# thangvubk/SoftGroup

Measured on AMD Instinct MI355X. Metric: scans/sec ScanNet-v2-like inference (softgroup_scannet.yaml, full forward_test), higher is better.
Workload: dtype f32

## Files before the change

softgroup_amd/csrc/radix_sort.h:

```cpp
#pragma once
#include <mutex>

#include "common.h"
#include "scan.h"

namespace sg {

constexpr int kRsBlock = 256;
constexpr int kRsItems = 8;
constexpr int kRsTile = kRsBlock * kRsItems;
constexpr int kRsBuckets = 256;

inline size_t radix_sort_workspace_bytes(int64_t n) {
  const int64_t nblk = (n + kRsTile - 1) / kRsTile;
  const int64_t hist = nblk * kRsBuckets + 1;
  return align_up(hist * 4) + align_up(scan_workspace_bytes(hist) + 4 * kRsBuckets * 4) +
         2 * align_up(n * 4) + 256;
}

static __global__ void __launch_bounds__(kRsBlock) rs_hist_kernel(const uint32_t *__restrict__ keys,
                                                          int64_t n, int shift, int nblk, int items,
                                                          int32_t *__restrict__ hist,
                                                          int32_t *totals) {
  __shared__ int h[kRsBuckets];
// ... 99 lines not shown
  }
  __syncthreads();
  for (int e = threadIdx.x; e < in_tile; e += kRsBlock) {
    const uint32_t key = skey[e];
    const int d = (key >> shift) & 0xff;
    const int off = base[d] + (e - dstart[d]);
    keys_out[off] = key;
    vals_out[off] = sval[e];
  }
}


static inline int radix_sort_pairs(uint32_t *keys, int32_t *vals, int64_t n, int num_bits, void *ws,
                            size_t ws_bytes, hipStream_t stream, uint32_t **keys_sorted,
                            int32_t **vals_sorted) {
  *keys_sorted = keys;
  *vals_sorted = vals;
  if (n <= 1 || num_bits <= 0) return SG_OK;
  if (ws_bytes < radix_sort_workspace_bytes(n)) {
    set_error("radix_sort_pairs: workspace too small");
    return SG_ERR_WORKSPACE;
  }
  int items = kRsItems;
  while (items < 64 && (n + static_cast<int64_t>(items) * kRsBlock - 1) / (static_cast<int64_t>(items) * kRsBlock) > 256)
    items *= 2;
  const int64_t tile = static_cast<int64_t>(items) * kRsBlock;
  const int nblk = static_cast<int>((n + tile - 1) / tile);
  const size_t lds = static_cast<size_t>(tile) * 8;
  {
    static std::mutex mu;
    static uint64_t done_mask = 0;
    int dev = 0;
    hipGetDevice(&dev);
    std::lock_guard<std::mutex> g(mu);
    if (dev < 0 || dev >= 64 || !((done_mask >> dev) & 1)) {
      if (hipFuncSetAttribute(reinterpret_cast<const void *>(rs_scatter_kernel),
                              hipFuncAttributeMaxDynamicSharedMemorySize, 64 * kRsBlock * 8) != hipSuccess) {
        (void)hipGetLastError();
        set_error("radix_sort_pairs: %d bytes of dynamic LDS are not available on this device (gfx950: 160 KB "
                  "per workgroup)", 64 * kRsBlock * 8);
        return SG_ERR_LAUNCH;
      }
      if (dev >= 0 && dev < 64) done_mask |= 1ull << dev;
    }
  }
  const int64_t hist_n = static_cast<int64_t>(nblk) * kRsBuckets;
  Workspace a(ws, ws_bytes);
  int32_t *hist = a.take<int32_t>(hist_n + 1);
  const size_t sbytes = scan_workspace_bytes(hist_n) + 4 * kRsBuckets * 4;
  void *sws = a.take<char>(sbytes);
  uint32_t *k2 = a.take<uint32_t>(n);
  int32_t *v2 = a.take<int32_t>(n);
  uint32_t *kin = keys, *kout = k2;
  int32_t *vin = vals, *vout = v2;
  const int n_pass = (num_bits + 7) / 8;
  const bool local_scan = nblk <= 256 && n_pass <= 4;
  int32_t *totals = static_cast<int32_t *>(sws);
  if (local_scan) hipMemsetAsync(totals, 0, static_cast<size_t>(n_pass) * kRsBuckets * 4, stream);
  for (int shift = 0, pass = 0; shift < num_bits; shift += 8, ++pass) {
    if (local_scan) {
      int32_t *t = totals + pass * kRsBuckets;
      rs_hist_kernel<<<nblk, kRsBlock, 0, stream>>>(kin, n, shift, nblk, items, hist, t);
      rs_scatter_kernel<<<nblk, kRsBlock, lds, stream>>>(kin, vin, n, shift, nblk, items, hist, t, kout, vout);
      if (const int rc = check_launch("radix_sort_pairs(scatter)"); rc != SG_OK) return rc;
    } else {
      rs_hist_kernel<<<nblk, kRsBlock, 0, stream>>>(kin, n, shift, nblk, items, hist, nullptr);
      int32_t *h = hist;
      int rc = exclusive_scan([h] __device__(int64_t i) { return h[i]; },
                              [h] __device__(int64_t i, int v) { h[i] = v; }, hist_n, nullptr, sws,
                              sbytes, stream);
      if (rc != SG_OK) return rc;
      rs_scatter_kernel<<<nblk, kRsBlock, lds, stream>>>(kin, vin, n, shift, nblk, items, hist, nullptr,
                                                         kout, vout);
      if (const int rc = check_launch("radix_sort_pairs(scatter)"); rc != SG_OK) return rc;
    }
    uint32_t *tk = kin; kin = kout; kout = tk;
    int32_t *tv = vin; vin = vout; vout = tv;
  }
  *keys_sorted = kin;
  *vals_sorted = vin;
  return check_launch("radix_sort_pairs");
}

}
```

softgroup_amd/csrc/spconv_rulebook.hip:

```cpp
#include <stdlib.h>

#include <mutex>

#include "common.h"
#include "radix_sort.h"
#include "scan.h"

namespace sg {

constexpr uint64_t kKeyEmpty = ~0ULL;

struct HashWs {
  uint64_t *keys;
  int32_t *vals;
  int32_t *owner, *rank;
  void *scan_ws;
  size_t scan_bytes;
  uint32_t cap;
};

static size_t hash_cap(int n) {
  size_t cap = 1024;
  while (cap < static_cast<size_t>(n) * 2) cap <<= 1;
  return cap;
// ... 186 lines not shown
    const int sl = slot[t];
    if (sl < 0 || vals[static_cast<size_t>(l) * cap + sl] != i) continue;
    const int r = pos[t] - pos[static_cast<size_t>(l) * M0];
    rowtab[static_cast<size_t>(l) * cap + sl] = r;
    const int4 c = reinterpret_cast<const int4 *>(indices0)[i];
    if (o.indices[l] != nullptr)
      reinterpret_cast<int4 *>(o.indices[l])[r] = make_int4(c.x, c.y >> l, c.z >> l, c.w >> l);
  }
}

__global__ void __launch_bounds__(256) pyr_link_kernel(const int32_t *__restrict__ indices0, int M0,
                                                      int L, const int32_t *__restrict__ vals,
                                                      const int32_t *__restrict__ rowtab,
                                                      uint32_t cap, const int32_t *__restrict__ slot,
                                                      const int32_t *__restrict__ pos, PyrOut o) {
  const int64_t total = static_cast<int64_t>(L - 1) * M0;
  for (int64_t t = blockIdx.x * 256LL + threadIdx.x; t < total; t += gridDim.x * 256LL) {
    const int l = static_cast<int>(t / M0), i = static_cast<int>(t - static_cast<int64_t>(l) * M0);
    const int sl = slot[t];
    if (sl < 0 || vals[static_cast<size_t>(l) * cap + sl] != i) continue;
    const int j = pos[t] - pos[static_cast<size_t>(l) * M0];
    const int s2 = slot[t + M0];
    const int up = s2 >= 0 ? rowtab[static_cast<size_t>(l + 1) * cap + s2] : -1;
    const int4 c = reinterpret_cast<const int4 *>(indices0)[i];
    const int k = (((c.y >> l) & 1) << 2) | (((c.z >> l) & 1) << 1) | ((c.w >> l) & 1);
    o.in2out[l][j] = up;
    if (up >= 0) o.child[l][static_cast<int64_t>(up) * 8 + k] = j;
    int4 *dst = reinterpret_cast<int4 *>(o.inv[l] + static_cast<int64_t>(j) * 8);
    dst[0] = make_int4(k == 0 ? up : -1, k == 1 ? up : -1, k == 2 ? up : -1, k == 3 ? up : -1);
    dst[1] = make_int4(k == 4 ? up : -1, k == 5 ? up : -1, k == 6 ? up : -1, k == 7 ? up : -1);
  }
}

__global__ void __launch_bounds__(256) pyr_subm_kernel(int L, const uint64_t *__restrict__ keys,
                                                      const int32_t *__restrict__ rowtab,
                                                      uint32_t cap, PyrOut o) {
  const long long total = o.pre27[L];
  int l = 0;
  for (long long t = blockIdx.x * 256LL + threadIdx.x; t < total; t += gridDim.x * 256LL) {
    while (t >= o.pre27[l + 1]) ++l;
    const long long e = t - o.pre27[l];
    const int j = static_cast<int>(e / 27), k = static_cast<int>(e - static_cast<long long>(j) * 27);
    const int4 c = reinterpret_cast<const int4 *>(o.indices[l])[j];
    const Shape3 s = o.shape[l];
    const int x = c.y + k / 9 - 1, y = c.z + (k / 3) % 3 - 1, z = c.w + k % 3 - 1;
    int32_t r = -1;
    if (k == 13) r = j;
    else if (x >= 0 && y >= 0 && z >= 0 && x < s.s0 && y < s.s1 && z < s.s2)
      r = hash_find(keys + static_cast<size_t>(l) * cap, rowtab + static_cast<size_t>(l) * cap, cap - 1,
                    lin_key(c.x, x, y, z, s));
    o.nbr[l][e] = r;
  }
}

struct PlanSeg {
  const int32_t *nbr;
  int32_t *order;
  uint32_t *tile_mask;
  int32_t *nbr_tiles;
  int rows, K, row_base, tile_base, sb_base, sb_rows;
  int key_bits, seg_code;
  const uint32_t *key_sorted;
  const int32_t *val_sorted;
};
struct PlanSegs {
  int n, total_rows, total_tiles, total_sbs;
  int n_big, big_rows;
  int n_wide, wide_rows;
  PlanSeg s[kPyrMaxSegs];
};

constexpr int kSbRowsMax = 16384;
constexpr int kSbIndexBits = 14;
static int plan_sb_rows(int rows) {
  static const int env = getenv("SG_PLAN_SB") ? atoi(getenv("SG_PLAN_SB")) : 0;
  int sb = env > 0 ? env : (rows + 7) / 8;
  if (env <= 0 && sb < 4096) sb = 4096;
  sb = (sb + 31) / 32 * 32;
  if (sb < 32) sb = 32;
  if (sb > kSbRowsMax) sb = kSbRowsMax;
  return sb;
}

__global__ void __launch_bounds__(1024) plan_sort_sb_kernel(PlanSegs P, const uint32_t *__restrict__ mask,
                                                           const int32_t *__restrict__ bitpos,
                                                           int32_t *__restrict__ val_sorted,
                                                           uint32_t *__restrict__ tmask) {
  extern __shared__ __attribute__((aligned(16))) uint64_t e[];
  __shared__ int pos[32];
  int seg = P.n_big;
  while (seg + 1 < P.n && static_cast<int>(blockIdx.x) >= P.s[seg + 1].sb_base) ++seg;
  const PlanSeg &S = P.s[seg];
  const int sb = blockIdx.x - S.sb_base;
  const int first = sb * S.sb_rows;
  const int cnt = min(S.sb_rows, S.rows - first);
  const int K = S.K;
  if (threadIdx.x < 32) pos[threadIdx.x] = bitpos[seg * 32 + threadIdx.x];
  int N = 64;
  while (N < cnt) N <<= 1;
  __syncthreads();
  for (int i = threadIdx.x; i < N; i += 1024) {
    uint64_t v = ~0ull;
    if (i < cnt) {
      uint32_t key = 0;
      for (uint32_t mm = mask[S.row_base + first + i]; mm; mm &= mm - 1) key |= 1u << pos[__ffs(static_cast<int>(mm)) - 1];
      v = (static_cast<uint64_t>(key) << kSbIndexBits) | static_cast<uint64_t>(i);
    }
    e[i] = v;
  }
  __syncthreads();
  for (int k = 2; k <= N; k <<= 1) {
    for (int j = k >> 1; j > 0; j >>= 1) {
      for (int t = threadIdx.x; t < N / 2; t += 1024) {
        const int i = 2 * t - (t & (j - 1));
        const int l = i + j;
        const uint64_t a = e[i], b = e[l];
        const bool up = (i & k) == 0;
        if ((a > b) == up) { e[i] = b; e[l] = a; }
      }
      __syncthreads();
    }
  }
  for (int i0 = 0; i0 < N; i0 += 1024) {
    const int i = i0 + threadIdx.x;
    uint32_t key = 0;
    if (i < cnt) {
      const uint64_t v = e[i];
      val_sorted[S.row_base + first + i] = first + static_cast<int>(v & ((1u << kSbIndexBits) - 1u));
      key = static_cast<uint32_t>(v >> kSbIndexBits);
    }
#pragma unroll
    for (int o = 16; o > 0; o >>= 1) key |= __shfl_xor(key, o, 64);
    if ((threadIdx.x & 31) == 0 && i < cnt) {
      uint32_t m = 0;
      for (int k = 0; k < K; ++k) m |= ((key >> pos[k]) & 1u) << k;
      tmask[S.tile_base + sb * (S.sb_rows >> 5) + (i >> 5)] = m;
    }
  }
}

__global__ void __launch_bounds__(1024) plan_tile_order_xcd_kernel(PlanSegs P, const uint32_t *__restrict__ tmask,
                                                                  int mode, int32_t *__restrict__ torder) {
  __shared__ int bucket[4096];
  __shared__ int hist[33];
  const PlanSeg &S = P.s[blockIdx.x];
  const int nt = (S.rows + 31) / 32;
  const int x = blockIdx.y, q = nt >> 3, r = nt & 7;
  const int cnt = q + (x < r ? 1 : 0), start = x * q + min(x, r);
  if (x == 0) {
    if (threadIdx.x < 33) hist[threadIdx.x] = 0;
    __syncthreads();
    for (int t = threadIdx.x; t < nt; t += 1024) atomicAdd(&hist[__popc(tmask[S.tile_base + t])], 1);
    __syncthreads();
    if (threadIdx.x < SG_PLAN_HIST_WORDS) S.tile_mask[nt + threadIdx.x] = threadIdx.x < 33 ? hist[threadIdx.x] : 0;
  }
  const int sb_tiles = S.sb_rows >> 5;
  const int sb0 = start / sb_tiles;
  auto bucket_of = [&](int t) {
    const int b = 32 - __popc(tmask[S.tile_base + t]);
    return mode == 2 ? (t / sb_tiles - sb0) * 33 + b : b;
  };
  for (int c0 = 0; c0 < cnt; c0 += 4096) {
    const int n = min(4096, cnt - c0);
    __syncthreads();
    for (int i = threadIdx.x; i < n; i += 1024) bucket[i] = bucket_of(start + c0 + i);
    __syncthreads();
    for (int i = threadIdx.x; i < n; i += 1024) {
      const int bi = bucket[i];
      int rank = 0;
      for (int j = 0; j < n; ++j) {
        const int bj = bucket[j];
        rank += (bj < bi || (bj == bi && j < i)) ? 1 : 0;
      }
      torder[S.tile_base + (c0 + rank) * 8 + x] = start + c0 + i;
    }
  }
}

__global__ void __launch_bounds__(256) plan_mask_all_kernel(PlanSegs P, uint32_t *__restrict__ mask,
                                                           int32_t *__restrict__ val,
                                                           int32_t *__restrict__ freq) {
  __shared__ int cnt[32];
  const int seg = blockIdx.y;
  const int rows = P.s[seg].rows, K = P.s[seg].K, row_base = P.s[seg].row_base;
  if (blockIdx.x * 256 >= rows) return;
  const int32_t *nbr = P.s[seg].nbr;
  if (threadIdx.x < 32) cnt[threadIdx.x] = 0;
  __syncthreads();
  const int j = blockIdx.x * 256 + threadIdx.x;
  uint32_t m = 0;
  if (j < rows) {
    const int32_t *row = nbr + static_cast<int64_t>(j) * K;
    for (int k = 0; k < K; ++k) m |= (row[k] >= 0 ? 1u : 0u) << k;
    mask[row_base + j] = m;
    val[row_base + j] = row_base + j;
  }
  for (int k = 0; k < K; ++k) {
    const int c = __popcll(__ballot((m >> k) & 1u));
    if ((threadIdx.x & 63) == 0 && c) atomicAdd(&cnt[k], c);
  }
  __syncthreads();
  if (threadIdx.x < K && cnt[threadIdx.x]) atomicAdd(&freq[seg * 32 + threadIdx.x], cnt[threadIdx.x]);
}

__global__ void plan_pos_all_kernel(PlanSegs P, const int32_t *__restrict__ freq, int32_t *__restrict__ bitpos) {
  const int seg = blockIdx.x, k = threadIdx.x;
  const int K = P.s[seg].K;
  int p = 0;
  if (k < K) {
    const int fk = freq[seg * 32 + k];
    for (int o = 0; o < K; ++o) {
      const int fo = freq[seg * 32 + o];
      p += (fo > fk || (fo == fk && o < k)) ? 1 : 0;
    }
  }
  bitpos[seg * 32 + k] = p;
}

__global__ void __launch_bounds__(256) plan_key_all_kernel(PlanSegs P, const int32_t *__restrict__ bitpos,
                                                          uint32_t *__restrict__ mask_to_key) {
  __shared__ int pos[32];
  const int seg = blockIdx.y;
  const int rows = P.s[seg].rows;
  if (blockIdx.x * 256 >= rows) return;
  if (threadIdx.x < 32) pos[threadIdx.x] = bitpos[seg * 32 + threadIdx.x];
  __syncthreads();
  const int j = blockIdx.x * 256 + threadIdx.x;
  if (j >= rows) return;
  const int g = P.s[seg].row_base + j;
  uint32_t key = 0;
  for (uint32_t mm = mask_to_key[g]; mm; mm &= mm - 1) key |= 1u << pos[__ffs(static_cast<int>(mm)) - 1];
  mask_to_key[g] = key | (static_cast<uint32_t>(P.s[seg].seg_code) << P.s[seg].key_bits);
}

__global__ void __launch_bounds__(256) plan_tiles_all_kernel(PlanSegs P, const int32_t *__restrict__ bitpos,
                                                            uint32_t *__restrict__ tmask) {
  __shared__ int pos[32];
  const int seg = blockIdx.y;
  const int rows = P.s[seg].rows, K = P.s[seg].K;
  if (blockIdx.x * 256 >= rows) return;
  if (threadIdx.x < 32) pos[threadIdx.x] = bitpos[seg * 32 + threadIdx.x];
  __syncthreads();
  const int j = blockIdx.x * 256 + threadIdx.x;
  uint32_t key = j < rows ? P.s[seg].key_sorted[P.s[seg].row_base + j] & ((1u << P.s[seg].key_bits) - 1u) : 0u;
#pragma unroll
  for (int o = 16; o > 0; o >>= 1) key |= __shfl_xor(key, o, 64);
  if ((threadIdx.x & 31) == 0 && j < rows) {
    uint32_t m = 0;
    for (int k = 0; k < K; ++k) m |= ((key >> pos[k]) & 1u) << k;
    tmask[P.s[seg].tile_base + (j >> 5)] = m;
  }
}

__global__ void __launch_bounds__(1024) plan_tile_order_all_kernel(PlanSegs P, const uint32_t *__restrict__ tmask,
                                                                  int32_t *__restrict__ torder) {
  __shared__ int hist[33], base[33];
  __shared__ int wcnt[16][33];
  const PlanSeg &S = P.s[blockIdx.x];
  const int nt = (S.rows + 31) / 32;
  const int wave = threadIdx.x >> 6, lane = threadIdx.x & 63;
  if (threadIdx.x < 33) hist[threadIdx.x] = 0;
  __syncthreads();
  for (int t = threadIdx.x; t < nt; t += 1024) atomicAdd(&hist[__popc(tmask[S.tile_base + t])], 1);
  __syncthreads();
  if (threadIdx.x == 0) {
    int run = 0;
    for (int b = 32; b >= 0; --b) { base[b] = run; run += hist[b]; }
  }
  if (threadIdx.x < SG_PLAN_HIST_WORDS) S.tile_mask[nt + threadIdx.x] = threadIdx.x < 33 ? hist[threadIdx.x] : 0;
  __syncthreads();
  for (int t0 = 0; t0 < nt; t0 += 1024) {
    if (threadIdx.x < 16 * 33) (&wcnt[0][0])[threadIdx.x] = 0;
    __syncthreads();
    const int t = t0 + threadIdx.x;
    const bool valid = t < nt;
    const int b = valid ? __popc(tmask[S.tile_base + t]) : 0;
    uint64_t peers = __ballot(valid);
#pragma unroll
    for (int bit = 0; bit < 6; ++bit) {
      const uint64_t bal = __ballot((b >> bit) & 1);
      peers &= ((b >> bit) & 1) ? bal : ~bal;
    }
    const int lane_rank = __popcll(peers & ((1ull << lane) - 1ull));
    if (valid && lane_rank == 0) wcnt[wave][b] = __popcll(peers);
    __syncthreads();
    if (valid) {
      int off = base[b] + lane_rank;
      for (int w = 0; w < wave; ++w) off += wcnt[w][b];
      torder[S.tile_base + off] = t;
    }
    __syncthreads();
    if (threadIdx.x < 33) {
      int add = 0;
      for (int w = 0; w < 16; ++w) add += wcnt[w][threadIdx.x];
      base[threadIdx.x] += add;
    }
    __syncthreads();
  }
}

__global__ void __launch_bounds__(256) plan_emit_all_kernel(PlanSegs P, const int32_t *__restrict__ val_local,
                                                           const uint32_t *__restrict__ tmask,
                                                           const int32_t *__restrict__ torder) {
  const int seg = blockIdx.y;
  const int rows = P.s[seg].rows, K = P.s[seg].K, tile_base = P.s[seg].tile_base;
  const int val_base = P.s[seg].row_base;
  const bool local_vals = seg >= P.n_big;
  const int32_t *val_sorted = local_vals ? val_local : P.s[seg].val_sorted;
  const int row_base = local_vals ? 0 : val_base;
  const int nt = (rows + 31) / 32, per_tile = 32 * K;
  const int32_t *nbr = P.s[seg].nbr;
  int32_t *order = P.s[seg].order, *nbr_tiles = P.s[seg].nbr_tiles;
  uint32_t *tile_mask = P.s[seg].tile_mask;
  for (int t2 = blockIdx.x; t2 < nt; t2 += gridDim.x) {
    const int t = torder[tile_base + t2];
    if (threadIdx.x == 0) tile_mask[t2] = tmask[tile_base + t];
    if (threadIdx.x < 32) {
      const int pos = t * 32 + threadIdx.x;
      order[t2 * 32 + threadIdx.x] = pos < rows ? val_sorted[val_base + pos] - row_base : -1;
    }
    for (int e = threadIdx.x; e < per_tile; e += 256) {
      const int r = e / K, k = e - r * K;
      const int pos = t * 32 + r;
      nbr_tiles[static_cast<int64_t>(t2) * per_tile + e] =
          pos < rows ? nbr[static_cast<int64_t>(val_sorted[val_base + pos] - row_base) * K + k] : -1;
    }
  }
}

static size_t plan_scratch_bytes(size_t R, size_t T) {
  return 2 * align_up(R * 4) + 2 * align_up(T * 4) + 2 * align_up(kPyrMaxSegs * 32 * 4) +
         radix_sort_workspace_bytes(static_cast<int64_t>(R)) + 512;
}

static int plan_order_mode() {
  static const int mode = getenv("SG_PLAN_ORDER") ? atoi(getenv("SG_PLAN_ORDER")) : 0;
  return mode;
}
static void finalize_segs(PlanSegs &P) {
  const int mode = plan_order_mode();
  PlanSeg big[kPyrMaxSegs], small[kPyrMaxSegs];
  int nb = 0, ns = 0;
  P.n_wide = 0;
  P.wide_rows = 0;
  if (mode == 0) {
    for (int i = 0; i < P.n; ++i)
      if (P.s[i].K > 8) big[nb++] = P.s[i];
    P.n_wide = nb;
    for (int i = 0; i < P.n; ++i)
      if (P.s[i].K <= 8) big[nb++] = P.s[i];
    for (int i = 0; i < nb; ++i) {
      big[i].key_bits = i < P.n_wide ? static_cast<int>(kPlanKeyBits) : 8;
      big[i].seg_code = i < P.n_wide ? i : i - P.n_wide;
    }
  } else {
    for (int i = 0; i < P.n; ++i) small[ns++] = P.s[i];
  }
  int row_base = 0, tile_base = 0, sb_base = 0;
  P.n_big = nb;
  for (int i = 0; i < P.n; ++i) {
    PlanSeg &S = P.s[i];
    S = i < nb ? big[i] : small[i - nb];
    S.row_base = row_base;
    S.tile_base = tile_base;
    S.sb_base = sb_base;
    S.sb_rows = mode == 0 ? (S.rows + 31) / 32 * 32 : plan_sb_rows(S.rows);
    row_base += S.rows;
    tile_base += (S.rows + 31) / 32;
    if (i >= nb) sb_base += (S.rows + S.sb_rows - 1) / S.sb_rows;
    if (i + 1 == nb) P.big_rows = row_base;
    if (i + 1 == P.n_wide) P.wide_rows = row_base;
  }
  if (nb == 0) P.big_rows = 0;
  P.total_rows = row_base;
  P.total_tiles = tile_base;
  P.total_sbs = sb_base;
}

static int build_plans(const PlanSegs &P, void *ws2, size_t ws2_bytes, bool zero_freq, hipStream_t stream,
                       const char *who) {
  Workspace wsp(ws2, ws2_bytes);
  const size_t R = static_cast<size_t>(P.total_rows);
  uint32_t *mask = wsp.take<uint32_t>(R);
  int32_t *val = wsp.take<int32_t>(R);
  uint32_t *tmask = wsp.take<uint32_t>(P.total_tiles);
  int32_t *torder = wsp.take<int32_t>(P.total_tiles);
  int32_t *freq = wsp.take<int32_t>(kPyrMaxSegs * 32);
  int32_t *bitpos = wsp.take<int32_t>(kPyrMaxSegs * 32);
  const size_t rs_bytes = radix_sort_workspace_bytes(static_cast<int64_t>(R));
  void *rs_ws = wsp.take<char>(rs_bytes);
  if (!rs_ws) {
    set_error("%s: build workspace too small", who);
    return SG_ERR_WORKSPACE;
  }
  if (zero_freq) hipMemsetAsync(freq, 0, kPyrMaxSegs * 32 * 4, stream);
  int max_rows = 0, max_big = 0;
  for (int i = 0; i < P.n; ++i) {
    max_rows = P.s[i].rows > max_rows ? P.s[i].rows : max_rows;
    if (i < P.n_big) max_big = P.s[i].rows > max_big ? P.s[i].rows : max_big;
  }
  const dim3 grid((max_rows + 255) / 256, P.n);
  plan_mask_all_kernel<<<grid, 256, 0, stream>>>(P, mask, val, freq);
  static const bool raw_env = getenv("SG_PLAN_RAW") != nullptr;
  if (raw_env) hipMemsetAsync(freq, 0, kPyrMaxSegs * 32 * 4, stream);
  plan_pos_all_kernel<<<P.n, 32, 0, stream>>>(P, freq, bitpos);
  const int mode = plan_order_mode();
  PlanSegs Q = P;
  if (P.n_big > 0) {
    const dim3 gbig((max_big + 255) / 256, P.n_big);
    plan_key_all_kernel<<<gbig, 256, 0, stream>>>(P, bitpos, mask);
    struct Group { int first, count, row0, rows, key_bits; } groups[2] = {
        {0, P.n_wide, 0, P.wide_rows, static_cast<int>(kPlanKeyBits)},
        {P.n_wide, P.n_big - P.n_wide, P.wide_rows, P.big_rows - P.wide_rows, 8}};
    for (const Group &g : groups) {
      if (g.count == 0 || g.rows == 0) continue;
      int nbits = g.key_bits;
      for (int n = g.count - 1; n > 0; n >>= 1) ++nbits;
      uint32_t *ms;
      int32_t *vs;
      int rc = radix_sort_pairs(mask + g.row0, val + g.row0, static_cast<int64_t>(g.rows), nbits, rs_ws, rs_bytes,
                                stream, &ms, &vs);
      if (rc != SG_OK) return rc;
      if (ms != mask + g.row0) {
        hipMemcpyAsync(mask + g.row0, ms, static_cast<size_t>(g.rows) * 4, hipMemcpyDeviceToDevice, stream);
        hipMemcpyAsync(val + g.row0, vs, static_cast<size_t>(g.rows) * 4, hipMemcpyDeviceToDevice, stream);
      }
      for (int i = g.first; i < g.first + g.count; ++i) {
        Q.s[i].key_sorted = mask;
        Q.s[i].val_sorted = val;
      }
    }
    plan_tiles_all_kernel<<<gbig, 256, 0, stream>>>(Q, bitpos, tmask);
  }
  if (P.total_sbs > 0) {
    int max_sb = 64;
    for (int i = P.n_big; i < P.n; ++i)
      while (max_sb < P.s[i].sb_rows && max_sb < P.s[i].rows) max_sb <<= 1;
    static std::once_flag once;
    std::call_once(once, [] {
      hipFuncSetAttribute(reinterpret_cast<const void *>(plan_sort_sb_kernel), hipFuncAttributeMaxDynamicSharedMemorySize,
                          kSbRowsMax * 8);
    });
    plan_sort_sb_kernel<<<P.total_sbs, 1024, static_cast<size_t>(max_sb) * 8, stream>>>(Q, mask, bitpos, val, tmask);
  }
  if (mode == 0) plan_tile_order_all_kernel<<<P.n, 1024, 0, stream>>>(Q, tmask, torder);
  else plan_tile_order_xcd_kernel<<<dim3(P.n, 8), 1024, 0, stream>>>(Q, tmask, mode, torder);
  plan_emit_all_kernel<<<dim3(min((max_rows + 31) / 32, 2048), P.n), 256, 0, stream>>>(Q, val, tmask, torder);
  return check_launch(who);
}

struct PyrWs {
  uint64_t *keys;
  int32_t *vals;
  int32_t *rowtab;
  int32_t *slot;
  int32_t *pos;
  void *scan_ws;
  size_t scan_bytes;
  uint32_t cap;
};
static bool pyr_carve(void *ws, size_t ws_bytes, int M0, int L, PyrWs *w) {
  Workspace a(ws, ws_bytes);
  const size_t nn = static_cast<size_t>(M0 > 0 ? M0 : 1);
  w->cap = static_cast<uint32_t>(hash_cap(M0));
  w->keys = a.take<uint64_t>(static_cast<size_t>(L) * w->cap);
  w->vals = a.take<int32_t>(static_cast<size_t>(L) * w->cap);
  w->rowtab = a.take<int32_t>(static_cast<size_t>(L) * w->cap);
  w->slot = a.take<int32_t>(static_cast<size_t>(L) * nn);
  w->pos = a.take<int32_t>(static_cast<size_t>(L) * nn + 1);
  w->scan_bytes = scan_workspace_bytes(static_cast<int64_t>(L) * nn);
  w->scan_ws = a.take<char>(w->scan_bytes);
  return w->scan_ws != nullptr;
}

}

using namespace sg;

extern "C" {

size_t sg_spconv_hash_workspace_bytes(int M) {
  const size_t nn = static_cast<size_t>(M > 0 ? M : 1);
  return align_up(hash_cap(M) * 8) + align_up(hash_cap(M) * 4) + 3 * align_up(nn * 4) +
         align_up(scan_workspace_bytes(M)) + 256;
}

static int build_hash_common(HashWs *w, void *ws, size_t ws_bytes, int M, hipStream_t stream,
                             const char *who) {
  if (!hash_carve(ws, ws_bytes, M, w)) {
    set_error("%s: workspace too small", who);
    return SG_ERR_WORKSPACE;
  }
  hipMemsetAsync(w->keys, 0xff, static_cast<size_t>(w->cap) * 8, stream);
  hipMemsetAsync(w->vals, 0x7f, static_cast<size_t>(w->cap) * 4, stream);
  return SG_OK;
}

int sg_spconv_subm_rulebook(const int32_t *indices, int M, const int32_t *shape_host, int32_t *nbr,
                            void *ws, size_t ws_bytes, sg_stream_t stream_) {
  SG_REQUIRE(M >= 0 && shape_host, "sg_spconv_subm_rulebook: bad arguments");
  if (M == 0) return SG_OK;
  hipStream_t stream = as_stream(stream_);
  HashWs w;
  int rc = build_hash_common(&w, ws, ws_bytes, M, stream, "sg_spconv_subm_rulebook");
  if (rc != SG_OK) return rc;
  const Shape3 shape{shape_host[0], shape_host[1], shape_host[2]};
  subm_insert_kernel<<<(M + 255) / 256, 256, 0, stream>>>(indices, M, shape, w.keys, w.vals,
                                                         w.cap - 1);
  subm_lookup_kernel<<<grid_for(static_cast<int64_t>(M) * 27, 256, 256 * 32), 256, 0, stream>>>(
      indices, M, shape, w.keys, w.vals, w.cap - 1, nbr);
  return check_launch("sg_spconv_subm_rulebook");
}

int sg_spconv_down_build(const int32_t *indices, int M, const int32_t *shape_host, int32_t *in2out,
                         int32_t *meta, void *ws, size_t ws_bytes, sg_stream_t stream_) {
  SG_REQUIRE(M >= 0 && shape_host, "sg_spconv_down_build: bad arguments");
  hipStream_t stream = as_stream(stream_);
  hipMemsetAsync(meta, 0, 4, stream);
  if (M == 0) return SG_OK;
  HashWs w;
  int rc = build_hash_common(&w, ws, ws_bytes, M, stream, "sg_spconv_down_build");
  if (rc != SG_OK) return rc;
  const Shape3 oshape{shape_host[0] / 2, shape_host[1] / 2, shape_host[2] / 2};
  const int grid = (M + 255) / 256;
  int32_t *slot_of = w.rank;
  down_insert_kernel<<<grid, 256, 0, stream>>>(indices, M, oshape, w.keys, w.vals, w.cap - 1,
// ... 73 lines not shown
  const int m0 = M0;
  const uint32_t cap = w.cap;
  const int64_t n = static_cast<int64_t>(L) * M0;
  int rc = exclusive_scan(
      [slot, vals, m0, cap] __device__(int64_t t) {
        const int64_t l = t / m0;
        const int sl = slot[t];
        return (sl >= 0 && vals[l * cap + sl] == static_cast<int32_t>(t - l * m0)) ? 1 : 0;
      },
      [pos] __device__(int64_t t, int v) { pos[t] = v; }, n, pos + n, w.scan_ws, w.scan_bytes, stream);
  if (rc != SG_OK) return rc;
  pyr_rows_kernel<<<1, 64, 0, stream>>>(w.pos, M0, L, rows_dev);
  return check_launch("sg_spconv_pyramid_rows");
}

static long long pyr_seg_rows(const sg_pyramid_level *lv, int L, int seg_kind, int l) {
  return seg_kind == 1 ? lv[l + 1].rows : lv[l].rows;
}

size_t sg_spconv_pyramid_build_workspace_bytes(const sg_pyramid_level *levels, int n_levels) {
  long long total = 0;
  for (int l = 0; l < n_levels; ++l) {
    total += levels[l].rows;
    if (l + 1 < n_levels) total += levels[l + 1].rows + levels[l].rows;
  }
  const size_t R = static_cast<size_t>(total > 0 ? total : 1);
  const size_t T = R / 32 + static_cast<size_t>(3 * n_levels) + 1;
  return plan_scratch_bytes(R, T);
}

int sg_spconv_pyramid_build(const int32_t *indices, int M0, const int32_t *shape_host, int n_levels,
                            const sg_pyramid_level *levels, void *ws, size_t ws_bytes, void *ws2,
                            size_t ws2_bytes, sg_stream_t stream_) {
  SG_REQUIRE(M0 >= 0 && shape_host && levels && n_levels >= 1 && n_levels <= kPyrMaxLevels,
             "sg_spconv_pyramid_build: bad arguments (M0=%d n_levels=%d)", M0, n_levels);
  SG_REQUIRE(levels[0].rows == M0, "sg_spconv_pyramid_build: levels[0].rows must be num_rows");
  if (M0 == 0) return SG_OK;
  hipStream_t stream = as_stream(stream_);
  const int L = n_levels;
  PyrWs w;
  if (!pyr_carve(ws, ws_bytes, M0, L, &w)) {
    set_error("sg_spconv_pyramid_build: workspace too small (%zu bytes)", ws_bytes);
    return SG_ERR_WORKSPACE;
  }
  SG_REQUIRE(ws2 != nullptr && ws2_bytes >= sg_spconv_pyramid_build_workspace_bytes(levels, L),
             "sg_spconv_pyramid_build: build workspace too small (%zu bytes)", ws2_bytes);
  PyrOut o;
  PlanSegs P;
  P.n = 0;
  auto add_seg = [&](const int32_t *nbr, int rows, int K, const sg_plan_ptrs &pl) {
    PlanSeg &S = P.s[P.n++];
    S.nbr = nbr; S.order = pl.order; S.tile_mask = pl.tile_mask; S.nbr_tiles = pl.nbr_tiles;
    S.rows = rows; S.K = K;
  };
  Shape3 s{shape_host[0], shape_host[1], shape_host[2]};
  o.pre27[0] = 0;
  for (int l = 0; l < kPyrMaxLevels; ++l) {
    const bool in = l < L;
    o.indices[l] = in ? levels[l].indices : nullptr;
    o.nbr[l] = in ? levels[l].nbr : nullptr;
    o.in2out[l] = in ? levels[l].in2out : nullptr;
    o.child[l] = in ? levels[l].child : nullptr;
    o.inv[l] = in ? levels[l].inv : nullptr;
    o.shape[l] = s;
    o.pre27[l + 1] = o.pre27[l] + (in ? static_cast<long long>(levels[l].rows) * 27 : 0);
    s = Shape3{s.s0 / 2, s.s1 / 2, s.s2 / 2};
  }
  for (int l = 0; l < L; ++l) {
    SG_REQUIRE(levels[l].rows >= 0 && levels[l].nbr && levels[l].indices && levels[l].subm.order,
               "sg_spconv_pyramid_build: level %d: missing output pointers", l);
    if (l + 1 < L)
      SG_REQUIRE(levels[l].in2out && levels[l].child && levels[l].inv && levels[l].down.order &&
                     levels[l].up.order, "sg_spconv_pyramid_build: level %d: missing output pointers", l);
  }
  for (int l = 0; l < L; ++l) {
    if (levels[l].rows > 0) add_seg(levels[l].nbr, levels[l].rows, 27, levels[l].subm);
    if (l + 1 < L) {
      if (levels[l + 1].rows > 0) add_seg(levels[l].child, levels[l + 1].rows, 8, levels[l].down);
      if (levels[l].rows > 0) add_seg(levels[l].inv, levels[l].rows, 8, levels[l].up);
    }
  }
  if (P.n == 0) return check_launch("sg_spconv_pyramid_build");
  finalize_segs(P);
  int32_t *freq;
  {
    Workspace wsp(ws2, ws2_bytes);
    const size_t R = static_cast<size_t>(P.total_rows);
    wsp.take<uint32_t>(R);
    wsp.take<int32_t>(R);
    wsp.take<uint32_t>(P.total_tiles);
    wsp.take<int32_t>(P.total_tiles);
    freq = wsp.take<int32_t>(kPyrMaxSegs * 32);
    if (!freq) {
      set_error("sg_spconv_pyramid_build: build workspace too small");
      return SG_ERR_WORKSPACE;
    }
  }
  {
    static_assert(kPyrMaxLevels + 1 <= kFillMax, "one fill region per level + the histogram");
    FillList f;
    for (int l = 0; l + 1 < L; ++l)
      if (levels[l + 1].rows > 0) f.add(levels[l].child, static_cast<size_t>(levels[l + 1].rows) * 8 * 4, 0xff);
    f.add(freq, kPyrMaxSegs * 32 * 4, 0);
    fill_many(f, stream);
  }
  const int g_all = grid_for(static_cast<int64_t>(L) * M0, 256, 4096);
  pyr_emit_kernel<<<g_all, 256, 0, stream>>>(indices, M0, L, w.vals, w.rowtab, w.cap, w.slot, w.pos, o);
  if (L > 1) {
    pyr_link_kernel<<<grid_for(static_cast<int64_t>(L - 1) * M0, 256, 4096), 256, 0, stream>>>(
        indices, M0, L, w.vals, w.rowtab, w.cap, w.slot, w.pos, o);
  }
  pyr_subm_kernel<<<grid_for(o.pre27[L], 256, 8192), 256, 0, stream>>>(L, w.keys, w.rowtab, w.cap, o);
  return build_plans(P, ws2, ws2_bytes, false, stream, "sg_spconv_pyramid_build");
}

size_t sg_spconv_plan_workspace_bytes(int M) {
  const size_t nn = static_cast<size_t>(M > 0 ? M : 1);
  return plan_scratch_bytes(nn, (nn + 31) / 32 + 1);
}

int sg_spconv_plan(const int32_t *nbr, int M, int K, int32_t *order, uint32_t *tile_mask,
                   int32_t *nbr_tiles, void *ws, size_t ws_bytes, sg_stream_t stream_) {
  SG_REQUIRE(M >= 0 && K >= 1 && K <= 27, "sg_spconv_plan: bad arguments (M=%d K=%d)", M, K);
  if (M == 0) return SG_OK;
  PlanSegs P;
  P.n = 1;
  P.s[0] = PlanSeg{nbr, order, tile_mask, nbr_tiles, M, K, 0, 0, 0, 0, 0, 0, nullptr, nullptr};
  finalize_segs(P);
  return build_plans(P, ws, ws_bytes, true, as_stream(stream_), "sg_spconv_plan");
}

}
```

Measured before the change: 435.7.

## Use segmented radix sort for plan keys and fold bit-position kernel into consumers

Adds a segmented radix sort that sorts each plan segment's keys inside its own row range. This drops the segment-code high bits from the key, so fewer radix passes are needed and each pass uses 512 or 256 buckets. Per-segment totals are zeroed up front, in the existing fill for the pyramid build or in a memset otherwise. The separate plan_pos_all kernel is removed, and each consuming kernel now recomputes the frequency-ranked bit positions locally. The cost is a linear search over segments in every workgroup and redundant per-block rank computation.

Measured after the change: 437.0 (median of 3 runs). Within noise of the previous version (+0.3%).

```diff
diff --git a/softgroup_amd/csrc/radix_sort.h b/softgroup_amd/csrc/radix_sort.h
--- a/softgroup_amd/csrc/radix_sort.h
+++ b/softgroup_amd/csrc/radix_sort.h
@@ -205,4 +205,230 @@
   return check_launch("radix_sort_pairs");
 }
 
-}
+constexpr int kRsSegMax = 32;
+constexpr int kRsSegMaxWgs = 256;
+struct RsSegs {
+  int n, items;
+  int row0[kRsSegMax + 1];
+  int wg0[kRsSegMax + 1];
+};
+inline bool rs_segs_layout(const int *rows, int n, RsSegs *S) {
+  if (n < 1 || n > kRsSegMax) return false;
+  for (int items = kRsItems; items <= 64; items *= 2) {
+    const int64_t tile = static_cast<int64_t>(items) * kRsBlock;
+    int64_t wgs = 0, row = 0;
+    for (int s = 0; s < n; ++s) {
+      S->row0[s] = static_cast<int>(row);
+      S->wg0[s] = static_cast<int>(wgs);
+      row += rows[s];
+      wgs += (rows[s] + tile - 1) / tile;
+    }
+    if (row >= (1ll << 31)) return false;
+    S->row0[n] = static_cast<int>(row);
+    S->wg0[n] = static_cast<int>(wgs);
+    S->n = n;
+    S->items = items;
+    if (wgs <= kRsSegMaxWgs) return true;
+  }
+  return false;
+}
+inline size_t rs_seg_hist_words(int bits) { return static_cast<size_t>(kRsSegMaxWgs) << bits; }
+inline size_t rs_seg_total_words(int n_seg, int num_bits, int bits) {
+  return static_cast<size_t>((num_bits + bits - 1) / bits) * n_seg * (static_cast<size_t>(1) << bits);
+}
+
+template <int BITS>
+static __global__ void __launch_bounds__(kRsBlock) rs_seg_hist_kernel(const uint32_t *__restrict__ keys, RsSegs S,
+                                                                      int shift, int32_t *__restrict__ hist,
+                                                                      int32_t *totals) {
+  constexpr int NB = 1 << BITS, PER = NB / kRsBlock;
+  __shared__ int h[NB];
+#pragma unroll
+  for (int q = 0; q < PER; ++q) h[threadIdx.x + q * kRsBlock] = 0;
+  __syncthreads();
+  const int wg = blockIdx.x;
+  int s = 0;
+  while (s + 1 < S.n && wg >= S.wg0[s + 1]) ++s;
+  const int wl = wg - S.wg0[s], nblk = S.wg0[s + 1] - S.wg0[s];
+  const int tile = S.items * kRsBlock;
+  const int first = S.row0[s] + wl * tile;
+  const int end = min(first + tile, S.row0[s + 1]);
+  for (int i = first + threadIdx.x; i < end; i += kRsBlock) atomicAdd(&h[(keys[i] >> shift) & (NB - 1)], 1);
+  __syncthreads();
+#pragma unroll
+  for (int q = 0; q < PER; ++q) {
+    const int d = threadIdx.x + q * kRsBlock;
+    const int c = h[d];
+    hist[static_cast<int64_t>(NB) * S.wg0[s] + static_cast<int64_t>(d) * nblk + wl] = c;
+    if (c) atomicAdd(&totals[s * NB + d], c);
+  }
+}
+
+template <int BITS>
+static __global__ void __launch_bounds__(kRsBlock) rs_seg_scatter_kernel(const uint32_t *__restrict__ keys,
+                                                                         const int32_t *__restrict__ vals, RsSegs S,
+                                                                         int shift, const int32_t *__restrict__ hist,
+                                                                         const int32_t *__restrict__ totals,
+                                                                         uint32_t *__restrict__ keys_out,
+                                                                         int32_t *__restrict__ vals_out) {
+  constexpr int NB = 1 << BITS, PER = NB / kRsBlock;
+  extern __shared__ __attribute__((aligned(16))) unsigned char rs_lds[];
+  const int items = S.items;
+  uint32_t *skey = reinterpret_cast<uint32_t *>(rs_lds);
+  int32_t *sval = reinterpret_cast<int32_t *>(rs_lds) + items * kRsBlock;
+  __shared__ int base[NB];
+  __shared__ int dstart[NB];
+  __shared__ int run[NB];
+  __shared__ int wcnt[4][NB];
+  __shared__ int lds4[4];
+  const int wave = threadIdx.x >> 6, lane = threadIdx.x & 63;
+  const int wg = blockIdx.x;
+  int s = 0;
+  while (s + 1 < S.n && wg >= S.wg0[s + 1]) ++s;
+  const int wl = wg - S.wg0[s], nblk = S.wg0[s + 1] - S.wg0[s];
+  const int tile = S.row0[s] + wl * items * kRsBlock;
+  const int in_tile = min(items * kRsBlock, S.row0[s + 1] - tile);
+#pragma unroll
+  for (int q = 0; q < PER; ++q) run[threadIdx.x + q * kRsBlock] = 0;
+  __syncthreads();
+  for (int e = threadIdx.x; e < in_tile; e += kRsBlock) atomicAdd(&run[(keys[tile + e] >> shift) & (NB - 1)], 1);
+  __syncthreads();
+  {
+    int mine[PER], sum = 0;
+#pragma unroll
+    for (int q = 0; q < PER; ++q) { mine[q] = run[threadIdx.x * PER + q]; sum += mine[q]; }
+    int excl = block_incl_scan_256(sum, lds4, nullptr) - sum;
+#pragma unroll
+    for (int q = 0; q < PER; ++q) { dstart[threadIdx.x * PER + q] = excl; excl += mine[q]; }
+  }
+  {
+    int tot[PER], before[PER], sum = 0;
+#pragma unroll
+    for (int q = 0; q < PER; ++q) {
+      const int d = threadIdx.x * PER + q;
+      const int32_t *row = hist + static_cast<int64_t>(NB) * S.wg0[s] + static_cast<int64_t>(d) * nblk;
+      int bf = 0, b = 0;
+      for (; b + 16 <= wl; b += 16) {
+        int v[16];
+#pragma unroll
+        for (int u = 0; u < 16; ++u) v[u] = row[b + u];
+#pragma unroll
+        for (int u = 0; u < 16; ++u) bf += v[u];
+      }
+      for (; b < wl; ++b) bf += row[b];
+      before[q] = bf;
+      tot[q] = totals[s * NB + d];
+      sum += tot[q];
+    }
+    int excl = block_incl_scan_256(sum, lds4, nullptr) - sum;
+#pragma unroll
+    for (int q = 0; q < PER; ++q) { base[threadIdx.x * PER + q] = S.row0[s] + excl + before[q]; excl += tot[q]; }
+  }
+#pragma unroll
+  for (int q = 0; q < PER; ++q) run[threadIdx.x + q * kRsBlock] = 0;
+  __syncthreads();
+  uint32_t pk[8];
+  int32_t pv[8];
+  for (int r = 0; r < items; ++r) {
+    if ((r & 7) == 0) {
+#pragma unroll
+      for (int q = 0; q < 8; ++q) {
+        const int e = (r + q) * kRsBlock + threadIdx.x;
+        pk[q] = e < in_tile ? keys[tile + e] : 0u;
+        pv[q] = e < in_tile ? vals[tile + e] : 0;
+      }
+    }
+#pragma unroll
+    for (int w = 0; w < 4; ++w)
+#pragma unroll
+      for (int q = 0; q < PER; ++q) wcnt[w][threadIdx.x + q * kRsBlock] = 0;
+    __syncthreads();
+    const bool valid = r * kRsBlock + static_cast<int>(threadIdx.x) < in_tile;
+    uint32_t key = 0u;
+    int32_t val = 0;
+#pragma unroll
+    for (int q = 0; q < 8; ++q)
+      if ((r & 7) == q) { key = pk[q]; val = pv[q]; }
+    const int d = (key >> shift) & (NB - 1);
+    uint64_t peers = __ballot(valid);
+#pragma unroll
+    for (int b = 0; b < BITS; ++b) {
+      const uint64_t bal = __ballot((d >> b) & 1);
+      peers &= ((d >> b) & 1) ? bal : ~bal;
+    }
+    const int lane_rank = __popcll(peers & ((1ull << lane) - 1ull));
+    if (valid && lane_rank == 0) wcnt[wave][d] = __popcll(peers);
+    __syncthreads();
+    if (valid) {
+      int off = dstart[d] + run[d] + lane_rank;
+      for (int w = 0; w < wave; ++w) off += wcnt[w][d];
+      skey[off] = key;
+      sval[off] = val;
+    }
+    __syncthreads();
+#pragma unroll
+    for (int q = 0; q < PER; ++q) {
+      const int dd = threadIdx.x + q * kRsBlock;
+      run[dd] += wcnt[0][dd] + wcnt[1][dd] + wcnt[2][dd] + wcnt[3][dd];
+    }
+  }
+  __syncthreads();
+  const int seg_lo = S.row0[s], seg_hi = S.row0[s + 1];
+  for (int e = threadIdx.x; e < in_tile; e += kRsBlock) {
+    const uint32_t key = skey[e];
+    const int d = (key >> shift) & (NB - 1);
+    const int off = base[d] + (e - dstart[d]);
+    if (off >= seg_lo && off < seg_hi) {
+      keys_out[off] = key;
+      vals_out[off] = sval[e];
+    }
+  }
+}
+
+template <int BITS>
+static inline int radix_sort_pairs_segmented(uint32_t *keys, int32_t *vals, uint32_t *keys2, int32_t *vals2,
+                                             const RsSegs &S, int num_bits, int32_t *hist, int32_t *totals,
+                                             hipStream_t stream, uint32_t **keys_sorted, int32_t **vals_sorted) {
+  static_assert(BITS == 8 || BITS == 9, "256 or 512 buckets at 256 threads");
+  constexpr int NB = 1 << BITS;
+  *keys_sorted = keys;
+  *vals_sorted = vals;
+  if (S.row0[S.n] <= 0 || num_bits <= 0) return SG_OK;
+  const int nwg = S.wg0[S.n];
+  if (nwg < 1 || nwg > kRsSegMaxWgs || S.items > 64) {
+    set_error("radix_sort_pairs_segmented: %d workgroups of %d rounds", nwg, S.items);
+    return SG_ERR_ARG;
+  }
+  const size_t lds = static_cast<size_t>(S.items) * kRsBlock * 8;
+  {
+    static std::mutex mu;
+    static uint64_t done_mask = 0;
+    int dev = 0;
+    hipGetDevice(&dev);
+    std::lock_guard<std::mutex> g(mu);
+    if (dev < 0 || dev >= 64 || !((done_mask >> dev) & 1)) {
+      if (hipFuncSetAttribute(reinterpret_cast<const void *>(rs_seg_scatter_kernel<BITS>),
+                              hipFuncAttributeMaxDynamicSharedMemorySize, 64 * kRsBlock * 8) != hipSuccess) {
+        (void)hipGetLastError();
+        set_error("radix_sort_pairs_segmented: %d bytes of dynamic LDS are not available on this device",
+                  64 * kRsBlock * 8);
+        return SG_ERR_LAUNCH;
+      }
+      if (dev >= 0 && dev < 64) done_mask |= 1ull << dev;
+    }
+  }
+  uint32_t *kin = keys, *kout = keys2;
+  int32_t *vin = vals, *vout = vals2;
+  for (int shift = 0, pass = 0; shift < num_bits; shift += BITS, ++pass) {
+    int32_t *t = totals + static_cast<size_t>(pass) * S.n * NB;
+    rs_seg_hist_kernel<BITS><<<nwg, kRsBlock, 0, stream>>>(kin, S, shift, hist, t);
+    rs_seg_scatter_kernel<BITS><<<nwg, kRsBlock, lds, stream>>>(kin, vin, S, shift, hist, t, kout, vout);
+    uint32_t *tk = kin; kin = kout; kout = tk;
+    int32_t *tv = vin; vin = vout; vout = tv;
+  }
+  *keys_sorted = kin;
+  *vals_sorted = vin;
+  return check_launch("radix_sort_pairs_segmented");
+}
+
+}
diff --git a/softgroup_amd/csrc/spconv_rulebook.hip b/softgroup_amd/csrc/spconv_rulebook.hip
--- a/softgroup_amd/csrc/spconv_rulebook.hip
+++ b/softgroup_amd/csrc/spconv_rulebook.hip
@@ -292,8 +292,22 @@
   return sb;
 }
 
+__device__ __forceinline__ void plan_bit_positions(const int32_t *__restrict__ freq, int seg, int K, int *pos) {
+  const int k = threadIdx.x;
+  if (k >= 32) return;
+  int p = 0;
+  if (k < K) {
+    const int fk = freq[seg * 32 + k];
+    for (int o = 0; o < K; ++o) {
+      const int fo = freq[seg * 32 + o];
+      p += (fo > fk || (fo == fk && o < k)) ? 1 : 0;
+    }
+  }
+  pos[k] = p;
+}
+
 __global__ void __launch_bounds__(1024) plan_sort_sb_kernel(PlanSegs P, const uint32_t *__restrict__ mask,
-                                                           const int32_t *__restrict__ bitpos,
+                                                           const int32_t *__restrict__ freq,
                                                            int32_t *__restrict__ val_sorted,
                                                            uint32_t *__restrict__ tmask) {
   extern __shared__ __attribute__((aligned(16))) uint64_t e[];
@@ -305,7 +319,7 @@
   const int first = sb * S.sb_rows;
   const int cnt = min(S.sb_rows, S.rows - first);
   const int K = S.K;
-  if (threadIdx.x < 32) pos[threadIdx.x] = bitpos[seg * 32 + threadIdx.x];
+  plan_bit_positions(freq, seg, K, pos);
   int N = 64;
   while (N < cnt) N <<= 1;
   __syncthreads();
@@ -413,43 +427,29 @@
   if (threadIdx.x < K && cnt[threadIdx.x]) atomicAdd(&freq[seg * 32 + threadIdx.x], cnt[threadIdx.x]);
 }
 
-__global__ void plan_pos_all_kernel(PlanSegs P, const int32_t *__restrict__ freq, int32_t *__restrict__ bitpos) {
-  const int seg = blockIdx.x, k = threadIdx.x;
-  const int K = P.s[seg].K;
-  int p = 0;
-  if (k < K) {
-    const int fk = freq[seg * 32 + k];
-    for (int o = 0; o < K; ++o) {
-      const int fo = freq[seg * 32 + o];
-      p += (fo > fk || (fo == fk && o < k)) ? 1 : 0;
-    }
-  }
-  bitpos[seg * 32 + k] = p;
-}
-
-__global__ void __launch_bounds__(256) plan_key_all_kernel(PlanSegs P, const int32_t *__restrict__ bitpos,
+__global__ void __launch_bounds__(256) plan_key_all_kernel(PlanSegs P, const int32_t *__restrict__ freq, int add_code,
                                                           uint32_t *__restrict__ mask_to_key) {
   __shared__ int pos[32];
   const int seg = blockIdx.y;
   const int rows = P.s[seg].rows;
   if (blockIdx.x * 256 >= rows) return;
-  if (threadIdx.x < 32) pos[threadIdx.x] = bitpos[seg * 32 + threadIdx.x];
+  plan_bit_positions(freq, seg, P.s[seg].K, pos);
   __syncthreads();
   const int j = blockIdx.x * 256 + threadIdx.x;
   if (j >= rows) return;
   const int g = P.s[seg].row_base + j;
   uint32_t key = 0;
   for (uint32_t mm = mask_to_key[g]; mm; mm &= mm - 1) key |= 1u << pos[__ffs(static_cast<int>(mm)) - 1];
-  mask_to_key[g] = key | (static_cast<uint32_t>(P.s[seg].seg_code) << P.s[seg].key_bits);
-}
-
-__global__ void __launch_bounds__(256) plan_tiles_all_kernel(PlanSegs P, const int32_t *__restrict__ bitpos,
+  mask_to_key[g] = add_code ? key | (static_cast<uint32_t>(P.s[seg].seg_code) << P.s[seg].key_bits) : key;
+}
+
+__global__ void __launch_bounds__(256) plan_tiles_all_kernel(PlanSegs P, const int32_t *__restrict__ freq,
                                                             uint32_t *__restrict__ tmask) {
   __shared__ int pos[32];
   const int seg = blockIdx.y;
   const int rows = P.s[seg].rows, K = P.s[seg].K;
   if (blockIdx.x * 256 >= rows) return;
-  if (threadIdx.x < 32) pos[threadIdx.x] = bitpos[seg * 32 + threadIdx.x];
+  plan_bit_positions(freq, seg, K, pos);
   __syncthreads();
   const int j = blockIdx.x * 256 + threadIdx.x;
   uint32_t key = j < rows ? P.s[seg].key_sorted[P.s[seg].row_base + j] & ((1u << P.s[seg].key_bits) - 1u) : 0u;
@@ -538,9 +538,39 @@
   }
 }
 
+constexpr size_t kPlanTotalsWide = 3 * static_cast<size_t>(kPyrMaxLevels) * 512;
+constexpr size_t kPlanTotalsNarrow = 2 * static_cast<size_t>(kPyrMaxLevels) * 256;
+constexpr size_t kPlanClearWords = kPyrMaxSegs * 32 + kPlanTotalsWide + kPlanTotalsNarrow;
 static size_t plan_scratch_bytes(size_t R, size_t T) {
-  return 2 * align_up(R * 4) + 2 * align_up(T * 4) + 2 * align_up(kPyrMaxSegs * 32 * 4) +
+  return 2 * align_up(R * 4) + 2 * align_up(T * 4) + align_up(kPlanClearWords * 4) + align_up(rs_seg_hist_words(9) * 4) +
          radix_sort_workspace_bytes(static_cast<int64_t>(R)) + 512;
+}
+struct PlanScratch {
+  uint32_t *mask;
+  int32_t *val;
+  uint32_t *tmask;
+  int32_t *torder;
+  int32_t *clear;
+  int32_t *freq, *totals_wide, *totals_narrow;
+  int32_t *seg_hist;
+  void *rs_ws;
+  size_t rs_bytes;
+};
+static bool plan_carve(void *ws, size_t ws_bytes, size_t R, size_t T, PlanScratch *s) {
+  Workspace wsp(ws, ws_bytes);
+  s->mask = wsp.take<uint32_t>(R);
+  s->val = wsp.take<int32_t>(R);
+  s->tmask = wsp.take<uint32_t>(T);
+  s->torder = wsp.take<int32_t>(T);
+  s->clear = wsp.take<int32_t>(kPlanClearWords);
+  s->seg_hist = wsp.take<int32_t>(rs_seg_hist_words(9));
+  s->rs_bytes = radix_sort_workspace_bytes(static_cast<int64_t>(R));
+  s->rs_ws = wsp.take<char>(s->rs_bytes);
+  if (!s->rs_ws || !s->clear || !s->seg_hist) return false;
+  s->freq = s->clear;
+  s->totals_wide = s->clear + kPyrMaxSegs * 32;
+  s->totals_narrow = s->totals_wide + kPlanTotalsWide;
+  return true;
 }
 
 static int plan_order_mode() {
@@ -587,48 +617,68 @@
   P.total_sbs = sb_base;
 }
 
-static int build_plans(const PlanSegs &P, void *ws2, size_t ws2_bytes, bool zero_freq, hipStream_t stream,
+static int build_plans(const PlanSegs &P, void *ws2, size_t ws2_bytes, bool cleared, hipStream_t stream,
                        const char *who) {
-  Workspace wsp(ws2, ws2_bytes);
-  const size_t R = static_cast<size_t>(P.total_rows);
-  uint32_t *mask = wsp.take<uint32_t>(R);
-  int32_t *val = wsp.take<int32_t>(R);
-  uint32_t *tmask = wsp.take<uint32_t>(P.total_tiles);
-  int32_t *torder = wsp.take<int32_t>(P.total_tiles);
-  int32_t *freq = wsp.take<int32_t>(kPyrMaxSegs * 32);
-  int32_t *bitpos = wsp.take<int32_t>(kPyrMaxSegs * 32);
-  const size_t rs_bytes = radix_sort_workspace_bytes(static_cast<int64_t>(R));
-  void *rs_ws = wsp.take<char>(rs_bytes);
-  if (!rs_ws) {
+  PlanScratch sc;
+  if (!plan_carve(ws2, ws2_bytes, static_cast<size_t>(P.total_rows), static_cast<size_t>(P.total_tiles), &sc)) {
     set_error("%s: build workspace too small", who);
     return SG_ERR_WORKSPACE;
   }
-  if (zero_freq) hipMemsetAsync(freq, 0, kPyrMaxSegs * 32 * 4, stream);
+  uint32_t *mask = sc.mask, *tmask = sc.tmask;
+  int32_t *val = sc.val, *torder = sc.torder, *freq = sc.freq;
   int max_rows = 0, max_big = 0;
   for (int i = 0; i < P.n; ++i) {
     max_rows = P.s[i].rows > max_rows ? P.s[i].rows : max_rows;
     if (i < P.n_big) max_big = P.s[i].rows > max_big ? P.s[i].rows : max_big;
   }
+  if (!cleared) hipMemsetAsync(sc.clear, 0, kPlanClearWords * 4, stream);
   const dim3 grid((max_rows + 255) / 256, P.n);
   plan_mask_all_kernel<<<grid, 256, 0, stream>>>(P, mask, val, freq);
   static const bool raw_env = getenv("SG_PLAN_RAW") != nullptr;
   if (raw_env) hipMemsetAsync(freq, 0, kPyrMaxSegs * 32 * 4, stream);
-  plan_pos_all_kernel<<<P.n, 32, 0, stream>>>(P, freq, bitpos);
   const int mode = plan_order_mode();
   PlanSegs Q = P;
   if (P.n_big > 0) {
     const dim3 gbig((max_big + 255) / 256, P.n_big);
-    plan_key_all_kernel<<<gbig, 256, 0, stream>>>(P, bitpos, mask);
-    struct Group { int first, count, row0, rows, key_bits; } groups[2] = {
-        {0, P.n_wide, 0, P.wide_rows, static_cast<int>(kPlanKeyBits)},
-        {P.n_wide, P.n_big - P.n_wide, P.wide_rows, P.big_rows - P.wide_rows, 8}};
+    struct Group { int first, count, row0, rows, key_bits; RsSegs segs; } groups[2] = {
+        {0, P.n_wide, 0, P.wide_rows, static_cast<int>(kPlanKeyBits), {}},
+        {P.n_wide, P.n_big - P.n_wide, P.wide_rows, P.big_rows - P.wide_rows, 8, {}}};
+    bool segmented = true;
+    for (Group &g : groups) {
+      if (g.count == 0 || g.rows == 0) continue;
+      int rows[kRsSegMax];
+      if (g.count > kRsSegMax) { segmented = false; break; }
+      for (int i = 0; i < g.count; ++i) rows[i] = P.s[g.first + i].rows;
+      const bool wide = g.key_bits > 8;
+      segmented = segmented && rs_segs_layout(rows, g.count, &g.segs) &&
+                  rs_seg_total_words(g.count, g.key_bits, wide ? 9 : 8) <= (wide ? kPlanTotalsWide : kPlanTotalsNarrow);
+    }
+    plan_key_all_kernel<<<gbig, 256, 0, stream>>>(P, freq, segmented ? 0 : 1, mask);
+    Workspace second(sc.rs_ws, sc.rs_bytes);
+    uint32_t *mask2 = second.take<uint32_t>(static_cast<size_t>(P.total_rows));
+    int32_t *val2 = second.take<int32_t>(static_cast<size_t>(P.total_rows));
     for (const Group &g : groups) {
       if (g.count == 0 || g.rows == 0) continue;
+      uint32_t *ms;
+      int32_t *vs;
+      if (segmented) {
+        int rc;
+        if (g.key_bits > 8)
+          rc = radix_sort_pairs_segmented<9>(mask + g.row0, val + g.row0, mask2 + g.row0, val2 + g.row0, g.segs,
+                                             g.key_bits, sc.seg_hist, sc.totals_wide, stream, &ms, &vs);
+        else
+          rc = radix_sort_pairs_segmented<8>(mask + g.row0, val + g.row0, mask2 + g.row0, val2 + g.row0, g.segs,
+                                             g.key_bits, sc.seg_hist, sc.totals_narrow, stream, &ms, &vs);
+        if (rc != SG_OK) return rc;
+        for (int i = g.first; i < g.first + g.count; ++i) {
+          Q.s[i].key_sorted = ms - g.row0;
+          Q.s[i].val_sorted = vs - g.row0;
+        }
+        continue;
+      }
       int nbits = g.key_bits;
       for (int n = g.count - 1; n > 0; n >>= 1) ++nbits;
-      uint32_t *ms;
-      int32_t *vs;
-      int rc = radix_sort_pairs(mask + g.row0, val + g.row0, static_cast<int64_t>(g.rows), nbits, rs_ws, rs_bytes,
+      int rc = radix_sort_pairs(mask + g.row0, val + g.row0, static_cast<int64_t>(g.rows), nbits, sc.rs_ws, sc.rs_bytes,
                                 stream, &ms, &vs);
       if (rc != SG_OK) return rc;
       if (ms != mask + g.row0) {
@@ -640,7 +690,7 @@
         Q.s[i].val_sorted = val;
       }
     }
-    plan_tiles_all_kernel<<<gbig, 256, 0, stream>>>(Q, bitpos, tmask);
+    plan_tiles_all_kernel<<<gbig, 256, 0, stream>>>(Q, freq, tmask);
   }
   if (P.total_sbs > 0) {
     int max_sb = 64;
@@ -651,7 +701,7 @@
       hipFuncSetAttribute(reinterpret_cast<const void *>(plan_sort_sb_kernel), hipFuncAttributeMaxDynamicSharedMemorySize,
                           kSbRowsMax * 8);
     });
-    plan_sort_sb_kernel<<<P.total_sbs, 1024, static_cast<size_t>(max_sb) * 8, stream>>>(Q, mask, bitpos, val, tmask);
+    plan_sort_sb_kernel<<<P.total_sbs, 1024, static_cast<size_t>(max_sb) * 8, stream>>>(Q, mask, freq, val, tmask);
   }
   if (mode == 0) plan_tile_order_all_kernel<<<P.n, 1024, 0, stream>>>(Q, tmask, torder);
   else plan_tile_order_xcd_kernel<<<dim3(P.n, 8), 1024, 0, stream>>>(Q, tmask, mode, torder);
@@ -891,26 +941,17 @@
   }
   if (P.n == 0) return check_launch("sg_spconv_pyramid_build");
   finalize_segs(P);
-  int32_t *freq;
+  PlanScratch sc;
+  if (!plan_carve(ws2, ws2_bytes, static_cast<size_t>(P.total_rows), static_cast<size_t>(P.total_tiles), &sc)) {
+    set_error("sg_spconv_pyramid_build: build workspace too small");
+    return SG_ERR_WORKSPACE;
+  }
   {
-    Workspace wsp(ws2, ws2_bytes);
-    const size_t R = static_cast<size_t>(P.total_rows);
-    wsp.take<uint32_t>(R);
-    wsp.take<int32_t>(R);
-    wsp.take<uint32_t>(P.total_tiles);
-    wsp.take<int32_t>(P.total_tiles);
-    freq = wsp.take<int32_t>(kPyrMaxSegs * 32);
-    if (!freq) {
-      set_error("sg_spconv_pyramid_build: build workspace too small");
-      return SG_ERR_WORKSPACE;
-    }
-  }
-  {
-    static_assert(kPyrMaxLevels + 1 <= kFillMax, "one fill region per level + the histogram");
+    static_assert(kPyrMaxLevels + 1 <= kFillMax, "one fill region per level + the counts");
     FillList f;
     for (int l = 0; l + 1 < L; ++l)
       if (levels[l + 1].rows > 0) f.add(levels[l].child, static_cast<size_t>(levels[l + 1].rows) * 8 * 4, 0xff);
-    f.add(freq, kPyrMaxSegs * 32 * 4, 0);
+    f.add(sc.clear, kPlanClearWords * 4, 0);
     fill_many(f, stream);
   }
   const int g_all = grid_for(static_cast<int64_t>(L) * M0, 256, 4096);
@@ -920,7 +961,7 @@
         indices, M0, L, w.vals, w.rowtab, w.cap, w.slot, w.pos, o);
   }
   pyr_subm_kernel<<<grid_for(o.pre27[L], 256, 8192), 256, 0, stream>>>(L, w.keys, w.rowtab, w.cap, o);
-  return build_plans(P, ws2, ws2_bytes, false, stream, "sg_spconv_pyramid_build");
+  return build_plans(P, ws2, ws2_bytes, true, stream, "sg_spconv_pyramid_build");
 }
 
 size_t sg_spconv_plan_workspace_bytes(int M) {
@@ -936,7 +977,7 @@
   P.n = 1;
   P.s[0] = PlanSeg{nbr, order, tile_mask, nbr_tiles, M, K, 0, 0, 0, 0, 0, 0, nullptr, nullptr};
   finalize_segs(P);
-  return build_plans(P, ws, ws_bytes, true, as_stream(stream_), "sg_spconv_plan");
-}
-
-}
+  return build_plans(P, ws, ws_bytes, false, as_stream(stream_), "sg_spconv_plan");
+}
+
+}
```
